# GTEC-UDC/roskfpos

Hardware: AMD Instinct MI355X
Metric: EKF predict+update steps/s at 65536 tags x 8 anchors; RMS pos err vs CPU ref (higher is better)
Workload: dtype f64 arithmetic; f64 state and covariance, f32/int32 measurements in HBM (KFPOS_STORE_MIXED)

## Files before the change

### __graft_entry__.py

```python
from __future__ import annotations

import os
import shutil
import subprocess
import sys

ROOT = os.path.dirname(os.path.abspath(__file__))
CSRC = os.path.join(ROOT, "roskfpos_amd", "csrc")
HIP_LIB = os.path.join(CSRC, "libkfpos_hip.so")
ADAPTOR_DEMO = os.path.join(CSRC, "kfpos_replay")


def _stale(target, sources):
    if not os.path.exists(target):
        return True
    mt = os.path.getmtime(target)
    return any(os.path.getmtime(s) > mt for s in sources if os.path.exists(s))


def build(force: bool = False) -> None:
    jobs = str(min(8, os.cpu_count() or 1))
    res = subprocess.run(["make", "-s", "-j", jobs, "-C", CSRC] + (["-B"] if force else []) + ["all"],
                         capture_output=True, text=True)
    if res.returncode != 0:
        sys.stderr.write(res.stdout + res.stderr)
        raise subprocess.CalledProcessError(res.returncode, res.args)
    res = subprocess.run(["make", "-s", "-C", CSRC, "check"], capture_output=True, text=True)
    if res.returncode != 0:
        sys.stderr.write(res.stdout + res.stderr)
        if os.path.exists(HIP_LIB):
            os.remove(HIP_LIB)
        raise RuntimeError("a build-time performance rule is broken (scratch inside a loop / a kernel lost its second "
                           "wavefront per SIMD / the 9-state epoch loop waits for a memory operation just issued / a trip of its gain "
                           "iteration touches memory or branches too often / its epoch loop carries a covariance across the back-edge in "
                           "registers): " + (res.stdout + res.stderr).strip())
    subprocess.check_call(["make", "-s", "-C", os.path.join(ROOT, "oracle")] + (["-B"] if force else []))
    import glob
    core_headers = sorted(glob.glob(os.path.join(CSRC, "kfpos_core*.h"))) + [os.path.join(CSRC, "kfpos_p48.h")]
    emu_dir = os.path.join(ROOT, "tests", "emu")
    emu_so = os.path.join(emu_dir, "libkfpos_emu.so")
    if force or _stale(emu_so, [os.path.join(emu_dir, "kfpos_emu.cpp")] + core_headers):
        subprocess.check_call(["g++", "-O2", "-std=c++17", "-fPIC", "-shared", "-Wno-unknown-pragmas",
                               "-o", emu_so, os.path.join(emu_dir, "kfpos_emu.cpp")])
    fake_dir = os.path.join(ROOT, "tests", "fake_rccl")
    fake_so = os.path.join(fake_dir, "libfake_rccl.so")
    if force or _stale(fake_so, [os.path.join(fake_dir, "fake_rccl.cpp")]):
        subprocess.check_call([shutil.which("hipcc") or "/opt/rocm/bin/hipcc", "-O2", "-std=c++17", "-shared", "-fPIC",
                               "-o", fake_so, os.path.join(fake_dir, "fake_rccl.cpp"), "-lrt"])
    if ROOT not in sys.path:
        sys.path.insert(0, ROOT)
    import roskfpos_amd
    from roskfpos_amd import capi
    capi.load()


def smoke() -> None:
    if ROOT not in sys.path:
        sys.path.insert(0, ROOT)
    sys.path.insert(0, os.path.join(ROOT, "oracle"))
    import numpy as np
    from roskfpos_amd import capi
    from roskfpos_amd.synth import Workload
    import oracle_py

    T, A, S = 256, 8, 12
    w = Workload(T, A)
    for model in (capi.MODEL_TOA, capi.MODEL_TOA_IMU):
        bank = capi.KfposBank(model, T, w.anchors, init_pos=w.init_positions())
        orc = oracle_py.OracleBank(model, T, w.anchors, init_pos=w.init_positions(), n_threads=4)
        err, cov = w.err_est(), w.accel_cov()
        for s in range(S):
            r, a, dt = w.ranges_mm(s), w.accel(s), w.dt_of(s)
            if model == capi.MODEL_TOA_IMU:
                bank.step_toa_imu(r, err, a, cov, dt)
                orc.step_imu(a, cov, 0.0)
                orc.step_toa(r, err, dt)
            else:
                bank.step_toa(r, err, dt)
                orc.step_toa(r, err, dt)
        x, _, _ = bank.get_state()
        xo, _ = orc.get_state()
        rms = float(np.sqrt(((x[:, :3] - xo[:, :3]) ** 2).sum(1).mean()))
        print(f"smoke model={model}: RMS position difference vs oracle = {rms:.3e} m")
        assert rms <= 1e-6, rms
        bank.close()


if __name__ == "__main__":
    build()
    if len(sys.argv) > 1 and sys.argv[1] == "smoke":
        smoke()
```

### roskfpos_amd/csrc/kfpos_core.h

```cpp
#ifndef KFPOS_CORE_H
#define KFPOS_CORE_H

#include <math.h>
#include <stdint.h>

#ifndef KFPOS_HD
#define KFPOS_HD
#endif
#define KFPOS_FN KFPOS_HD inline __attribute__((always_inline))
#if defined(__clang__)
#define KFPOS_UNROLL _Pragma("unroll")
#define KFPOS_NOUNROLL _Pragma("nounroll")
#else
#define KFPOS_UNROLL
#define KFPOS_NOUNROLL
#endif

#if defined(__HIP_DEVICE_COMPILE__)
#define KFPOS_WAVE_ALL(pred) (__all((pred) ? 1 : 0) != 0)
#else
#define KFPOS_WAVE_ALL(pred) (pred)
#endif
#if defined(__HIP_DEVICE_COMPILE__)
#define KFPOS_WAVE_ANY(pred) (__builtin_amdgcn_ballot_w64(pred) != 0)
// ... 73 lines not shown
}
KFPOS_FN void kf_sqrt_rsqrt(double x, double &d, double &invd) {
#if defined(__HIP_DEVICE_COMPILE__)
    invd = kf_rsqrt(x);
    const double s = x * invd;
    d = __builtin_fma(__builtin_fma(-s, s, x) * 0.5, invd, s);
#else
    d = sqrt(x);
    invd = 1.0 / d;
#endif
}

KFPOS_FN void kf_sqrt_rsqrt_sweep(double x, double &d, double &invd) {
#if defined(__HIP_DEVICE_COMPILE__)
    double y = __builtin_amdgcn_rsq(x);
    const double e = __builtin_fma(-(0.5 * x) * y, y, 0.5);
    y = __builtin_fma(y, e, y);
    const double s = x * y;
    d = __builtin_fma(__builtin_fma(-s, s, x) * 0.5, y, s);
    invd = y;
#else
    d = sqrt(x);
    invd = 1.0 / d;
#endif
}

KFPOS_FN double kf_mm_to_m(int32_t mm) {
#if defined(__HIP_DEVICE_COMPILE__)
    const double x = (double)mm;
    const double q = x * 0.001;
    const double r = __builtin_fma(-q, 1000.0, x);
    return __builtin_fma(r, 0.001, q);
#else
    return (double)mm / 1000;
#endif
}

KFPOS_FN bool rel_change_below(double cost, double c, double tol) {
    const double lhs = fabs(cost - c), rhs = tol * cost;
    const bool clear = cost > 0.0 && fabs(lhs - rhs) > 1e-13 * rhs;
    if (KFPOS_WAVE_ALL(clear)) return lhs < rhs;
    return lhs / cost < tol;
}

KFPOS_FN bool rel_change_below_voted(double cost, double c, double tol) {
    const double lhs = fabs(cost - c), rhs = tol * cost;
    const bool clear = cost > 0.0 && fabs(lhs - rhs) > 1e-13 * rhs;
    bool below = lhs < rhs;
    if (KFPOS_WAVE_ANY(!clear)) below = lhs / cost < tol;
    return below;
}

KFPOS_FN bool rel_change_above(double cost, double c, double tol) {
    const double lhs = fabs(cost - c), rhs = tol * cost;
    const bool clear = cost > 0.0 && fabs(lhs - rhs) > 1e-13 * rhs;
    if (KFPOS_WAVE_ALL(clear)) return lhs > rhs;
    return lhs / cost > tol;
}

KFPOS_FN double stdmax(double a, double b) { return (a < b) ? b : a; }

template <int N, bool SYMM>
struct Cov {
    static constexpr int SZ = SYMM ? N * (N + 1) / 2 : N * N;
    double a[SZ];
    KFPOS_HD static constexpr int idx(int i, int j) {
        return SYMM ? (i <= j ? i * N - i * (i - 1) / 2 + (j - i) : j * N - j * (j - 1) / 2 + (i - j))
                    : i * N + j;
    }
    KFPOS_HD double operator()(int i, int j) const { return a[idx(i, j)]; }
    KFPOS_HD double &operator()(int i, int j) { return a[idx(i, j)]; }
};

struct Params {
    const double *anchors;
    int n_anchors;
    double accel_noise, jolt, cost_threshold;
    int ignore_worst, top_n, use_init_pos;
    int ml_variant = 0;
    int use_fixed_height, imu_fixed_cov_acc, imu_fixed_cov_w;
    double px4_height, px4_arm_p1, px4_arm_p2, px4_cov_vel, px4_cov_gyro_z;
    double imu_cov_acc, imu_cov_w, mag_offset, mag_cov;
    const double *pair_anchor_tab = nullptr;
};

KFPOS_FN double sym3_cofactors(const double h[6], double c[6]) {
    c[0] = h[3] * h[5] - h[4] * h[4];
    c[1] = h[2] * h[4] - h[1] * h[5];
    c[2] = h[1] * h[4] - h[2] * h[3];
    c[3] = h[0] * h[5] - h[2] * h[2];
    c[4] = h[1] * h[2] - h[0] * h[4];
    c[5] = h[0] * h[3] - h[1] * h[1];
    return h[0] * c[0] + h[1] * c[1] + h[2] * c[2];
}
KFPOS_FN double gen3_adjugate(const double m[9], double adj[9]) {
    adj[0] = m[4] * m[8] - m[5] * m[7];
    adj[1] = m[2] * m[7] - m[1] * m[8];
    adj[2] = m[1] * m[5] - m[2] * m[4];
    adj[3] = m[5] * m[6] - m[3] * m[8];
    adj[4] = m[0] * m[8] - m[2] * m[6];
    adj[5] = m[2] * m[3] - m[0] * m[5];
    adj[6] = m[3] * m[7] - m[4] * m[6];
    adj[7] = m[1] * m[6] - m[0] * m[7];
    adj[8] = m[0] * m[4] - m[1] * m[3];
    return m[0] * adj[0] + m[1] * adj[3] + m[2] * adj[6];
}

template <int N, int K>
KFPOS_FN void gauss_solve(const double *a, const double *b, double *x) {
    double r[N][N + K];
    KFPOS_UNROLL
    for (int i = 0; i < N; ++i) {
        KFPOS_UNROLL
        for (int j = 0; j < N; ++j) r[i][j] = a[N * i + j];
        KFPOS_UNROLL
        for (int k = 0; k < K; ++k) r[i][N + k] = b[K * i + k];
    }
    KFPOS_UNROLL
    for (int c = 0; c < N; ++c) {
        KFPOS_UNROLL
        for (int i = c + 1; i < N; ++i) {
            const bool sw = fabs(r[i][c]) > fabs(r[c][c]);
            KFPOS_UNROLL
            for (int k = c; k < N + K; ++k) {
                const double tc = r[c][k], ti = r[i][k];
                r[c][k] = sw ? ti : tc;
                r[i][k] = sw ? tc : ti;
            }
        }
        const double ip = 1.0 / r[c][c];
        KFPOS_UNROLL
        for (int i = c + 1; i < N; ++i) {
            const double f = r[i][c] * ip;
            KFPOS_UNROLL
            for (int k = c + 1; k < N + K; ++k) r[i][k] -= f * r[c][k];
        }
    }
    KFPOS_UNROLL
    for (int k = 0; k < K; ++k) {
        double sol[N];
        KFPOS_UNROLL
        for (int i = N - 1; i >= 0; --i) {
            double v = r[i][N + k];
            KFPOS_UNROLL
            for (int j = i + 1; j < N; ++j) v -= r[i][j] * sol[j];
            sol[i] = v / r[i][i];
        }
        KFPOS_UNROLL
        for (int i = 0; i < N; ++i) x[K * i + k] = sol[i];
    }
}

KFPOS_FN void chol3_psd(const double m[6], double l[6], double il[3]) {
    const double REL = 1e-12;
    double d = m[0], sq, isq;
    bool ok = d > 0.0;
    kf_sqrt_rsqrt(ok ? d : 1.0, sq, isq);
    l[0] = ok ? sq : 0.0;
    il[0] = ok ? isq : 0.0;
    l[1] = m[1] * il[0];
    l[2] = m[2] * il[0];
    d = m[3] - l[1] * l[1];
    ok = d > REL * m[3];
    kf_sqrt_rsqrt(ok ? d : 1.0, sq, isq);
    l[3] = ok ? sq : 0.0;
    il[1] = ok ? isq : 0.0;
// ... 159 lines not shown
```

### roskfpos_amd/csrc/kfpos_core_imu9.h

```cpp
#ifndef KFPOS_CORE_IMU9_H
#define KFPOS_CORE_IMU9_H

namespace kfpos {

constexpr double INFO_FORM_MIN_PIVOT = 1e-7;

struct Tag9 {
    double pos[3], vel[3];
    Cov<9, true> P;
};
struct Imu {
    bool has;
    double acc[3];
    double *ci;
    int ci_stride;
    KFPOS_HD double Wi(int k) const { return ci[(6 + k) * ci_stride]; }
};

KFPOS_FN void imu_whitener(const double s[9], double *ci, int ci_stride) {
    double c00, c11, c22, i00, i11, i22;
    kf_sqrt_rsqrt(s[0], c00, i00);
    const double c10 = s[3] * i00, c20 = s[6] * i00;
    kf_sqrt_rsqrt(s[4] - c10 * c10, c11, i11);
    const double c21 = (s[7] - c20 * c10) * i11;
// ... 538 lines not shown
template <bool DIAG, bool ACC0>
KFPOS_FN void iekf9_pairs(uint64_t m, const double xhat[9], const double *binv, int binv_stride,
                          const RegScratch<8> &sc, const double *anchor_tab, const Imu &imu, int max_steps, double tol,
                          Iekf9Iter &it, Iekf9Out &o) {
    const int lane = (int)__builtin_amdgcn_mbcnt_hi(~0u, __builtin_amdgcn_mbcnt_lo(~0u, 0u));
    const int g = lane >> 1, h = lane & 1;
    const int n_surv = __popcll(m);
    bool act = g < n_surv;
    const int src = nth_set_bit(m, act ? g : 0);
    const int src4 = src << 2;
    double xh[9];
    KFPOS_UNROLL
    for (int k = 0; k < 3; ++k) {
        xh[k] = lane_pull(xhat[k], src4);
        xh[3 + k] = 0.0;
        xh[6 + k] = ACC0 ? 0.0 : lane_pull(xhat[6 + k], src4);
    }
    Iekf9Iter ct;
    KFPOS_UNROLL
    for (int k = 0; k < 6; ++k) { ct.ve[k] = lane_pull(it.ve[k], src4); ct.wl[k] = lane_pull(it.wl[k], src4); }
    ct.qd = lane_pull(it.qd, src4);
    ct.cost = lane_pull(it.cost, src4);
    Iekf9Out co;
    KFPOS_UNROLL
    for (int k = 0; k < 6; ++k) co.mrlast[k] = lane_pull(o.mrlast[k], src4);
    KFPOS_UNROLL
    for (int k = 0; k < 3; ++k) co.dlast[k] = lane_pull(o.dlast[k], src4);
    co.gain_iters = __builtin_amdgcn_ds_bpermute(src4, o.gain_iters);
    Imu ci;
    ci.has = __builtin_amdgcn_ds_bpermute(src4, imu.has ? 1 : 0) != 0;
    KFPOS_UNROLL
    for (int k = 0; k < 3; ++k) ci.acc[k] = lane_pull(imu.acc[k], src4);
    ci.ci = imu.ci + (src - lane);
    ci.ci_stride = imu.ci_stride;
    double r4[4], w4[4];
    KFPOS_UNROLL
    for (int k = 0; k < 4; ++k) {
        const double r0 = lane_pull(sc.r[k], src4), r1 = lane_pull(sc.r[4 + k], src4);
        const double w0 = lane_pull(sc.w[k], src4), w1 = lane_pull(sc.w[4 + k], src4);
        r4[k] = h ? r1 : r0;
        w4[k] = h ? w1 : w0;
    }
    const double *cbinv = binv + (src - lane);
    const double *b4 = anchor_tab + 12 * h;
    const double b0[3] = {b4[0], b4[1], b4[2]};
    while (act) {
        double bb[12];
        const int z = kf_opaque_zero();
        bb[0] = b0[0]; bb[1] = b0[1]; bb[2] = b0[2];
        KFPOS_UNROLL
        for (int k = 3; k < 12; ++k) bb[k] = b4[k + z];
        Iekf9Parked pk;
        iekf9_fetch<true, DIAG>(cbinv, binv_stride, ci, pk);
        const double p[3] = {xh[0] + ct.ve[0], xh[1] + ct.ve[1], xh[2] + ct.ve[2]};
        Sweep9 sw, other;
        iekf9_sweep4(p, r4, w4, bb, sw);
        other.c = dpp_exchange(sw.c, 0);
        KFPOS_UNROLL
        for (int k = 0; k < 6; ++k) other.m[k] = dpp_exchange(sw.m[k], 0);
        KFPOS_UNROLL
        for (int k = 0; k < 3; ++k) other.u[k] = dpp_exchange(sw.u[k], 0);
        sweep9_add(sw, other);
        iekf9_spread_reads();
        const bool more = iekf9_pass<DIAG, false>(xh, pk, ci, tol, sw, ct, co);
        act = more && co.gain_iters < max_steps;
    }
    const bool owner = (m >> lane) & 1ull;
    const int rank = __popcll(m & ((1ull << lane) - 1ull));
    const int from4 = (owner ? 2 * rank : lane) << 2;
    KFPOS_UNROLL
    for (int k = 0; k < 6; ++k) {
        const double a = lane_pull(ct.wl[k], from4), b = lane_pull(co.mrlast[k], from4);
        if (owner) { it.wl[k] = a; o.mrlast[k] = b; }
    }
    KFPOS_UNROLL
    for (int k = 0; k < 3; ++k) {
        const double a = lane_pull(co.dlast[k], from4);
        if (owner) o.dlast[k] = a;
    }
    const double cst = lane_pull(ct.cost, from4);
    const int gi = __builtin_amdgcn_ds_bpermute(from4, co.gain_iters);
    if (owner) { it.cost = cst; o.gain_iters = gi; }
}
#endif

template <bool DIAG, bool ALLIMU, bool RANGING, bool ACC0 = false, bool HOLD = true, bool SETTLE = false, class SC>
KFPOS_FN void iekf9_info(const double xhat[9], const double *binv, int binv_stride, SC &sc, const Params &pr,
                         const Imu &imu, int max_steps, double tol, Iekf9Out &o) {
    Iekf9Iter it;
    KFPOS_UNROLL
    for (int k = 0; k < 6; ++k) { it.ve[k] = 0.0; it.wl[k] = 0.0; o.mrlast[k] = 0.0; }
    it.qd = 0.0;
    it.cost = 1e20;
    o.dlast[0] = o.dlast[1] = o.dlast[2] = 0.0;
    o.gain_iters = 0;
#if defined(__HIP_DEVICE_COMPILE__)
    constexpr bool PAIRS = RANGING && SC::NA == 8 && SC::CHUNK == 0 && !SC::COOP;
    const bool pairs = PAIRS && pr.pair_anchor_tab && __builtin_amdgcn_ballot_w64(true) == ~0ull;
#endif
    bool more = true;
    int stop = max_steps;
#if defined(__HIP_DEVICE_COMPILE__)
    if (pairs) stop = 8 < max_steps ? 8 : max_steps;
#endif
    Iekf9Parked pk;
    if constexpr (HOLD) iekf9_fetch<false, DIAG, true>(binv, binv_stride, imu, pk);
#if defined(__HIP_DEVICE_COMPILE__)
    if constexpr (HOLD && SETTLE) __builtin_amdgcn_s_waitcnt(0xC07F);
#endif
    for (;;) {
        while (more && o.gain_iters < stop) {
            if constexpr (!HOLD) iekf9_fetch<false, DIAG, false>(binv, binv_stride, imu, pk);
            const double p[3] = {xhat[0] + it.ve[0], xhat[1] + it.ve[1], xhat[2] + it.ve[2]};
            Sweep9 sw;
            iekf9_sweep<RANGING>(p, sc, pr, sw);
            more = iekf9_pass<DIAG, ALLIMU>(xhat, pk, imu, tol, sw, it, o);
        }
#if defined(__HIP_DEVICE_COMPILE__)
        if constexpr (PAIRS) {
            if (pairs) {
                const uint64_t m = __builtin_amdgcn_ballot_w64(more && o.gain_iters < max_steps);
                if (m == 0) break;
                if (__popcll(m) <= 32) {
                    iekf9_pairs<DIAG, ACC0>(m, xhat, binv, binv_stride, sc, pr.pair_anchor_tab, imu, max_steps, tol, it, o);
                    break;
                }
                stop = stop + 4 < max_steps ? stop + 4 : max_steps;
                continue;
            }
        }
#endif
        break;
    }
    KFPOS_UNROLL
    for (int k = 0; k < 6; ++k) o.w[k] = it.wl[k];
    o.cost = it.cost;
}

KFPOS_FN void cov_update9(Cov<9, true> &P, const double mr[6], const double d[3], const Imu &imu) {
    Factor9 f;
    factor9(mr, d, imu, f);
    KFPOS_UNROLL
    for (int k = 0; k < 6; ++k) {
        double pt[9], s = 1.0;
        KFPOS_UNROLL
        for (int i = 0; i < 9; ++i) {
            double v = 0.0;
            KFPOS_UNROLL
            for (int l = 0; l < 6; ++l) {
                const bool nz = (l < 3 && k < 3 && l >= k) || (l >= 3 && k >= 3 && l <= k);
                if (nz) v += P(i, e9(l)) * L9(f, l, k);
            }
            pt[i] = v;
        }
        KFPOS_UNROLL
        for (int l = 0; l < 6; ++l) {
            const bool nz = (l < 3 && k < 3 && l >= k) || (l >= 3 && k >= 3 && l <= k);
            if (nz) s += L9(f, l, k) * pt[e9(l)];
        }
        const double is = kf_rcp(s);
        KFPOS_UNROLL
        for (int i = 0; i < 9; ++i) {
            const double pi = pt[i] * is;
            KFPOS_UNROLL
            for (int j = i; j < 9; ++j) P(i, j) -= pi * pt[j];
        }
    }
}

struct CovPark9 {
    double *a;
    int stride;
};

KFPOS_FN bool imu9_started(const Tag9 &tg, const Params &pr) {
    return pr.use_init_pos || !(isnan(tg.pos[0]) || isnan(tg.pos[1]));
}
template <bool RANGING, class SC>
KFPOS_FN bool imu9_ml_init(double pos[3], SC &sc, const Params &pr, int n_valid, double c[6], uint32_t &status) {
    status = 0;
    if (!RANGING) return false;
    status = ST_FEW_RANGES;
    if (n_valid < 4) return false;
    double p[3] = {1.0, 1.0, 4.0}, sse;
    set_weights_ml(sc, pr, 0ull);
    const int it = ml_estimate(p, sc, pr, 0, n_valid, sse);
    status = ST_UPDATE_SKIPPED;
    if (ml_covariance_throws(sc, pr, 0, n_valid, sse)) return false;
    if (!ml_covariance(p, sc, pr, sse, c)) return false;
    pos[0] = p[0]; pos[1] = p[1]; pos[2] = p[2];
    status = pack_status(ST_ML_INIT, 0, it, -1);
    return true;
}
KFPOS_FN void imu9_predict_state(const Tag9 &tg, double dt, double xhat[9]) {
    const double c = dt * dt / 2;
    KFPOS_UNROLL
    for (int k = 0; k < 3; ++k) {
        xhat[k] = tg.pos[k] + dt * tg.vel[k] + c * 0.0;
        xhat[3 + k] = tg.vel[k] + dt * 0.0;
        xhat[6 + k] = 0.0;
    }
}
KFPOS_FN void imu9_park(const Cov<9, true> &P, const CovPark9 &park) {
    KFPOS_UNROLL
    for (int k = 0; k < 45; ++k) park.a[k * park.stride] = P.a[k];
}
KFPOS_FN void imu9_unpark(Cov<9, true> &P, const CovPark9 &park) {
    KFPOS_UNROLL
    for (int k = 0; k < 45; ++k) P.a[k] = park.a[k * park.stride];
}
KFPOS_FN bool imu9_predict_park(Cov<9, true> &P, double dt, double jolt, const CovPark9 &park) {
    predict9(P, dt, jolt);
    Cov<6, true> B;
    KFPOS_UNROLL
    for (int i = 0; i < 6; ++i) {
        KFPOS_UNROLL
        for (int j = i; j < 6; ++j) B(i, j) = P(e9(i), e9(j));
    }
    imu9_park(P, park);
    return sym6_inverse(B, park.a + 45 * park.stride, park.stride, INFO_FORM_MIN_PIVOT);
}
template <bool RANGING, bool HOLD, bool SETTLE, class SC>
KFPOS_FN void imu9_iterate(Tag9 &tg, const double xhat[9], SC &sc, const Params &pr, const Imu &imu,
                           const CovPark9 &park, bool fast, bool invertible, Iekf9Out &o) {
    double *binv = park.a + 45 * park.stride;
    if (invertible) {
        if (fast) iekf9_info<true, true, RANGING, true, HOLD, SETTLE>(xhat, binv, park.stride, sc, pr, imu, 20, 1e-4, o);
        else iekf9_info<false, false, RANGING, true, HOLD, SETTLE>(xhat, binv, park.stride, sc, pr, imu, 20, 1e-4, o);
        imu9_unpark(tg.P, park);
    } else {
        imu9_unpark(tg.P, park);
        if (fast) iekf9<true, RANGING>(xhat, tg.P, sc, pr, imu, 20, 1e-4, o);
        else iekf9<false, RANGING>(xhat, tg.P, sc, pr, imu, 20, 1e-4, o);
    }
    KFPOS_UNROLL
    for (int i = 0; i < 6; ++i) {
        double v = 0.0;
        KFPOS_UNROLL
        for (int k = 0; k < 6; ++k) v += tg.P(i, e9(k)) * o.w[k];
        if (i < 3) tg.pos[i] = xhat[i] + v;
        else tg.vel[i - 3] = xhat[i] + v;
    }
}

template <bool RANGING, bool HOLD = true, class SC>
KFPOS_FN bool step_imu9_state(Tag9 &tg, SC &sc, const Params &pr, double dt, const Imu &imu, const CovPark9 &park,
                              bool fast, Iekf9Out &o, uint32_t &status) {
    constexpr bool has_ranging = RANGING;
    const int n_valid = has_ranging ? count_used(sc, pr, 0) : 0;
    if (!pr.use_init_pos && (isnan(tg.pos[0]) || isnan(tg.pos[1]))) {
        status = 0;
        if (!has_ranging) return false;
        status = ST_FEW_RANGES;
        if (n_valid < 4) return false;
        double p[3] = {1.0, 1.0, 4.0}, sse, c[6];
        set_weights_ml(sc, pr, 0ull);
        const int it = ml_estimate(p, sc, pr, 0, n_valid, sse);
        status = ST_UPDATE_SKIPPED;
        if (ml_covariance_throws(sc, pr, 0, n_valid, sse)) return false;
        if (!ml_covariance(p, sc, pr, sse, c)) return false;
        tg.pos[0] = p[0]; tg.pos[1] = p[1]; tg.pos[2] = p[2];
        tg.P(0, 0) = c[0]; tg.P(0, 1) = c[1]; tg.P(1, 1) = c[3];
        status = pack_status(ST_ML_INIT, 0, it, -1);
        return false;
    }
    const double c = dt * dt / 2;
    double xhat[9];
    KFPOS_UNROLL
    for (int k = 0; k < 3; ++k) {
        xhat[k] = tg.pos[k] + dt * tg.vel[k] + c * 0.0;
        xhat[3 + k] = tg.vel[k] + dt * 0.0;
        xhat[6 + k] = 0.0;
    }
    predict9(tg.P, dt, pr.jolt);
    Cov<6, true> B;
    KFPOS_UNROLL
    for (int i = 0; i < 6; ++i) {
        KFPOS_UNROLL
        for (int j = i; j < 6; ++j) B(i, j) = tg.P(e9(i), e9(j));
    }
    KFPOS_UNROLL
    for (int k = 0; k < 45; ++k) park.a[k * park.stride] = tg.P.a[k];
    double *binv = park.a + 45 * park.stride;
    const bool invertible = sym6_inverse(B, binv, park.stride, INFO_FORM_MIN_PIVOT);
    iekf9_weights(xhat, sc, pr, has_ranging, n_valid, o);
    if (o.flags & ST_UPDATE_SKIPPED) {
        KFPOS_UNROLL
        for (int k = 0; k < 45; ++k) tg.P.a[k] = park.a[k * park.stride];
        status = ST_UPDATE_SKIPPED;
        return false;
    }
    if (invertible) {
        if (fast) iekf9_info<true, true, RANGING, true, HOLD>(xhat, binv, park.stride, sc, pr, imu, 20, 1e-4, o);
        else iekf9_info<false, false, RANGING, true, HOLD>(xhat, binv, park.stride, sc, pr, imu, 20, 1e-4, o);
        KFPOS_UNROLL
        for (int k = 0; k < 45; ++k) tg.P.a[k] = park.a[k * park.stride];
    } else {
        KFPOS_UNROLL
        for (int k = 0; k < 45; ++k) tg.P.a[k] = park.a[k * park.stride];
        if (fast) iekf9<true, RANGING>(xhat, tg.P, sc, pr, imu, 20, 1e-4, o);
        else iekf9<false, RANGING>(xhat, tg.P, sc, pr, imu, 20, 1e-4, o);
    }
    KFPOS_UNROLL
    for (int i = 0; i < 6; ++i) {
        double v = 0.0;
        KFPOS_UNROLL
        for (int k = 0; k < 6; ++k) v += tg.P(i, e9(k)) * o.w[k];
        if (i < 3) tg.pos[i] = xhat[i] + v;
        else tg.vel[i - 3] = xhat[i] + v;
    }
    status = 0;
    return true;
}
KFPOS_FN bool step_imu9_head(Tag9 &tg, const Params &pr, double dt, const CovPark9 &park) {
    if (imu9_started(tg, pr)) return imu9_predict_park(tg.P, dt, pr.jolt, park);
    imu9_park(tg.P, park);
    return false;
}
template <bool RANGING, bool HOLD = true, class SC>
KFPOS_FN bool step_imu9_state_parked(Tag9 &tg, SC &sc, const Params &pr, double dt, const Imu &imu,
                                     const CovPark9 &park, bool fast, bool invertible, Iekf9Out &o, uint32_t &status) {
    constexpr bool has_ranging = RANGING;
    const int n_valid = has_ranging ? count_used(sc, pr, 0) : 0;
    if (!imu9_started(tg, pr)) {
        double c[6];
        if (imu9_ml_init<RANGING>(tg.pos, sc, pr, n_valid, c, status)) {
            park.a[Cov<9, true>::idx(0, 0) * park.stride] = c[0];
            park.a[Cov<9, true>::idx(0, 1) * park.stride] = c[1];
            park.a[Cov<9, true>::idx(1, 1) * park.stride] = c[3];
        }
        imu9_unpark(tg.P, park);
        return false;
    }
    double xhat[9];
    imu9_predict_state(tg, dt, xhat);
    iekf9_weights(xhat, sc, pr, has_ranging, n_valid, o);
    if (o.flags & ST_UPDATE_SKIPPED) {
        imu9_unpark(tg.P, park);
        status = ST_UPDATE_SKIPPED;
        return false;
    }
    imu9_iterate<RANGING, HOLD, true>(tg, xhat, sc, pr, imu, park, fast, invertible, o);
    status = 0;
    return true;
}
KFPOS_FN uint32_t step_imu9_cov(Tag9 &tg, const Iekf9Out &o, const Imu &imu) {
    cov_update9(tg.P, o.mrlast, o.dlast, imu);
    return pack_status(o.flags, o.gain_iters, o.ml_iters, -1);
}
template <bool RANGING, class SC>
KFPOS_FN uint32_t step_imu9(Tag9 &tg, SC &sc, const Params &pr, double dt, const Imu &imu, const CovPark9 &park) {
    Iekf9Out o;
    uint32_t status;
    if (!step_imu9_state<RANGING>(tg, sc, pr, dt, imu, park, false, o, status)) return status;
    return step_imu9_cov(tg, o, imu);
}

KFPOS_FN void pose9(const Tag9 &tg, double t, double jolt, double pos[3], double vel[3], double cov[9]) {
    const double c = t * t / 2, t3 = (t * t * t) / 6;
    KFPOS_UNROLL
    for (int i = 0; i < 3; ++i) {
        pos[i] = tg.pos[i] + t * tg.vel[i];
        vel[i] = tg.vel[i];
        KFPOS_UNROLL
        for (int j = 0; j < 3; ++j) {
            const Cov<9, true> &P = tg.P;
            const double xpp = P(i, j) + t * P(3 + i, j) + c * P(6 + i, j);
            const double xpv = P(i, 3 + j) + t * P(3 + i, 3 + j) + c * P(6 + i, 3 + j);
            const double xpa = P(i, 6 + j) + t * P(3 + i, 6 + j) + c * P(6 + i, 6 + j);
            cov[3 * i + j] = xpp + t * xpv + c * xpa + (i == j ? jolt * t3 * t3 : 0.0);
        }
    }
}

}
#endif
```

### roskfpos_amd/csrc/kfpos_hip.hip

```cpp
#include <algorithm>
#include <cmath>
#include <cstdio>
#include <cstdlib>
#include <cstring>
#include <new>
#include <string>
#include <type_traits>
#include <vector>

#include "kfpos_kernels.h"

std::string &kfpos_error_text() {
    thread_local std::string text;
    return text;
}

namespace {

#define g_err (kfpos_error_text())

#define HIPCHK(expr)                                                                              \
    do {                                                                                          \
        hipError_t e_ = (expr);                                                                   \
        if (e_ != hipSuccess) {                                                                   \
// ... 224 lines not shown
using DevScope = KfposDevScope;

inline int pidx(const kfpos_handle *h, int i, int j) {
    if (h->full) return i * h->n + j;
    const int N = h->n;
    if (i > j) { const int tt = i; i = j; j = tt; }
    return i * N - i * (i - 1) / 2 + (j - i);
}

}

extern "C" {

const char *kfpos_last_error(void) { return g_err.c_str(); }
const char *kfpos_strerror(int code) {
    switch (code) {
    case KFPOS_OK: return "ok";
    case KFPOS_ERR_ARG: return "invalid argument";
    case KFPOS_ERR_HIP: return "HIP runtime error";
    case KFPOS_ERR_NO_DEVICE: return "no usable GPU";
    case KFPOS_ERR_MODEL: return "call not defined for this model";
    case KFPOS_ERR_STATE: return "call out of sequence";
    case KFPOS_ERR_COMM: return "RCCL error";
    default: return "unknown error";
    }
}
int kfpos_version(void) { return KFPOS_VERSION; }

int kfpos_create(const kfpos_config *cfg, kfpos_handle **out) {
    if (!cfg || !out) return KFPOS_ERR_ARG;
    *out = nullptr;
    g_err.clear();
    auto bad = [](const char *why) {
        g_err = why;
        return KFPOS_ERR_ARG;
    };
    if (cfg->model != KFPOS_MODEL_TOA && cfg->model != KFPOS_MODEL_TOA_IMU && cfg->model != KFPOS_MODEL_ML &&
        cfg->model != KFPOS_MODEL_PLANAR)
        return bad("kfpos_config.model is not one of KFPOS_MODEL_*");
    if (cfg->storage != KFPOS_STORE_F64 && cfg->storage != KFPOS_STORE_F32 && cfg->storage != KFPOS_STORE_MIXED &&
        cfg->storage != KFPOS_STORE_P48)
        return bad("kfpos_config.storage is not one of KFPOS_STORE_*");
    if (cfg->n_tags < 1) return bad("kfpos_config.n_tags must be >= 1");
    if (cfg->max_anchors < 1 || cfg->max_anchors > KFPOS_MAX_ANCHORS)
        return bad("kfpos_config.max_anchors must be 1..64 (MAX_NUM_ANCS, Posgenerator.h:74)");
    if (cfg->top_n < 0) return bad("kfpos_config.top_n must be >= 0");
    if (cfg->ml_variant != KFPOS_ML_NORMAL && cfg->ml_variant != KFPOS_ML_IGNORE_N && cfg->ml_variant != KFPOS_ML_BEST)
        return bad("kfpos_config.ml_variant is not one of KFPOS_ML_*");
    if (cfg->ml_variant != KFPOS_ML_NORMAL && cfg->model != KFPOS_MODEL_ML)
        return bad("kfpos_config.ml_variant belongs to KFPOS_MODEL_ML (MLLocation's variants, MLLocation.h:5-7)");
    if ((cfg->model == KFPOS_MODEL_TOA_IMU && (cfg->top_n || cfg->ignore_worst)) ||
        (cfg->model == KFPOS_MODEL_ML && cfg->ignore_worst) ||
        (cfg->model == KFPOS_MODEL_PLANAR && (cfg->top_n || cfg->ignore_worst)))
        return bad("ignore_worst exists for the 6-state filter only, top_n for the 6-state filter and the ML estimator");
    int ndev = 0;
    if (hipGetDeviceCount(&ndev) != hipSuccess || ndev <= 0 || cfg->device < 0 || cfg->device >= ndev) {
        g_err = "no HIP device";
        return KFPOS_ERR_NO_DEVICE;
    }
    DevScope dev_(cfg->device);
    kfpos_handle *h = new (std::nothrow) kfpos_handle();
    if (!h) return KFPOS_ERR_ARG;
    h->cfg = *cfg;
    h->n = cfg->model == KFPOS_MODEL_TOA_IMU ? 9 : (cfg->model == KFPOS_MODEL_ML ? 3 : (cfg->model == KFPOS_MODEL_PLANAR ? 8 : 6));
    h->full = (cfg->model == KFPOS_MODEL_TOA && !cfg->use_init_pos) ? 1 : 0;
    h->psz = h->full ? h->n * h->n : h->n * (h->n + 1) / 2;
    h->rsz = cfg->storage == KFPOS_STORE_F32 ? 4 : (cfg->storage == KFPOS_STORE_P48 ? 6 : 8);
    h->msz = cfg->storage == KFPOS_STORE_F64 ? 8 : 4;
    h->A = 0;
    h->have_anchors = false;
    h->stepped = false;
    {
        const char *g = getenv("KFPOS_GENERIC_KERNEL");
        h->force_generic = g && g[0] == '1';
        if (h->full && cfg->ignore_worst && cfg->storage == KFPOS_STORE_P48) h->force_generic = true;
        {
            hipDeviceProp_t prop;
            const char *ow = getenv("KFPOS_ONE_WAVE_BUILD");
            h->two_waves = false;
            if (!(ow && ow[0] == '1') && hipGetDeviceProperties(&prop, cfg->device) == hipSuccess)
                h->two_waves = ((size_t)cfg->n_tags + WAVE - 1) / WAVE > (size_t)prop.multiProcessorCount * 4;
        }
        const char *np = getenv("KFPOS_PAIR9");
        h->pair9 = np && np[0] == '1';
        const char *nd = getenv("KFPOS_IMU9_DIAG");
        h->imu9_diag = !(nd && nd[0] == '0');
        const char *nc = getenv("KFPOS_NO_COOP");
        h->coop = !(nc && nc[0] == '1') && !h->force_generic && cfg->model == KFPOS_MODEL_TOA && cfg->use_init_pos &&
                  !cfg->ignore_worst && !cfg->top_n && cfg->max_anchors <= COOP_LANES && cfg->n_tags <= 8192;
        const char *c = getenv("KFPOS_TRACE_CHUNK_STEPS");
        int n = c ? atoi(c) : KFPOS_TRACE_CHUNK;
        h->trace_chunk = n < 1 ? 1 : (n > KFPOS_TRACE_CHUNK ? KFPOS_TRACE_CHUNK : n);
    }
    std::memset(h->anchors, 0, sizeof(h->anchors));
    const size_t T = cfg->n_tags, A = cfg->max_anchors, r = h->rsz, m = h->msz;
#define ALLOC(ptr, bytes)                                                     \
    do {                                                                      \
        hipError_t e_ = hipMalloc((void **)&(ptr), (bytes));                  \
        if (e_ != hipSuccess) {                                               \
            g_err = std::string("hipMalloc: ") + hipGetErrorString(e_);       \
            kfpos_destroy(h);                                                 \
            return KFPOS_ERR_HIP;                                             \
        }                                                                     \
        (void)hipMemset((ptr), 0, (bytes));                                   \
    } while (0)
    ALLOC(h->d_pos, 3 * T * sizeof(double));
    ALLOC(h->d_P, h->psz * T * r);
    ALLOC(h->d_flags, T * sizeof(uint32_t));
    if (h->n == 3) ALLOC(h->d_vel, 3 * T * sizeof(double));
    if (h->n == 8) {
        ALLOC(h->d_vel, 4 * T * sizeof(double));
        ALLOC(h->d_latch, LATCH_ROWS * T * sizeof(double));
        ALLOC(h->d_sensor, 24 * T * sizeof(double));
    }
    if (h->n == 9) {
        ALLOC(h->d_vel, 3 * T * sizeof(double));
        ALLOC(h->d_imu_acc, 3 * T * m);
        ALLOC(h->d_imu_cov, 6 * T * m);
        ALLOC(h->d_accel, 3 * T * m);
        ALLOC(h->d_cov, 9 * T * m);
    }
    ALLOC(h->d_ranges, A * T * sizeof(int32_t));
    ALLOC(h->d_err, A * T * m);
    ALLOC(h->d_dt, T * sizeof(double));
    ALLOC(h->d_out, 15 * T * sizeof(double));
    ALLOC(h->d_status, T * sizeof(uint32_t));
#undef ALLOC
    if (hipEventCreate(&h->ev0) != hipSuccess || hipEventCreate(&h->ev1) != hipSuccess) {
        g_err = "hipEventCreate failed";
        kfpos_destroy(h);
        return KFPOS_ERR_HIP;
    }
    if (T * A <= small_bank_limit()) {
        size_t off = 0;
        auto region = [&](size_t bytes) { const size_t o = off; off += (bytes + 255) & ~(size_t)255; return o; };
        h->sm_ranges = region(A * T * sizeof(int32_t));
        h->sm_err = region(A * T * m);
        h->sm_accel = region(3 * T * m);
        h->sm_cov = region(9 * T * m);
        h->sm_dt = region(T * sizeof(double));
        h->sm_sensor = region(24 * T * sizeof(double));
        h->sm_status = region(T * sizeof(uint32_t));
        h->sm_out = region((size_t)(15 + h->n + h->n * h->n) * T * sizeof(double));
        void *hp = nullptr, *dp = nullptr;
        if (hipHostMalloc(&hp, off, hipHostMallocMapped) != hipSuccess || hipHostGetDevicePointer(&dp, hp, 0) != hipSuccess) {
            g_err = "hipHostMalloc(mapped block of a small bank) failed";
            if (hp) (void)hipHostFree(hp);
            kfpos_destroy(h);
            return KFPOS_ERR_HIP;
        }
        std::memset(hp, 0, off);
        h->sm_h = (unsigned char *)hp;
        h->sm_bytes = off;
        h->sm_d = (unsigned char *)dp;
    }
    const bool parks = cfg->model == KFPOS_MODEL_PLANAR || (cfg->model == KFPOS_MODEL_TOA && h->full);
    if (cfg->model == KFPOS_MODEL_TOA_IMU && lds_bytes(h) + park9_bytes() > 64 * 1024) {
        hipError_t e_ = hipFuncSetAttribute((const void *)step_kernel(h), hipFuncAttributeMaxDynamicSharedMemorySize,
                                            (int)(lds_bytes(h) + park9_bytes()));
        if (e_ != hipSuccess) {
            g_err = std::string("hipFuncSetAttribute: ") + hipGetErrorString(e_);
            kfpos_destroy(h);
            return KFPOS_ERR_HIP;
        }
    } else if (lds_bytes(h) + (parks ? park_bytes() : 0) > 64 * 1024) {
        hipError_t e_ = hipFuncSetAttribute((const void *)step_kernel(h), hipFuncAttributeMaxDynamicSharedMemorySize,
                                            (int)(lds_bytes(h) + (h->full ? park_bytes() : 0)));
// ... 1986 lines not shown
```

### roskfpos_amd/csrc/kfpos_k_imu9.hip

```cpp
#include "kfpos_kernels.h"

namespace {

template <typename W>
__device__ inline void in_agpr(W &w) {
    static_assert(sizeof(W) == 4, "one register");
    asm volatile("" : "+a"(w));
}

__device__ inline void forget(double &v) { asm volatile("" : "=v"(v)); }

template <typename REAL, typename MREAL, int AS, bool RANGING = true>
__global__ __launch_bounds__(WAVE) void k_step_imu9(const KArgs a) {
    extern __shared__ double lds[];
    const int lane = threadIdx.x;
    const size_t t = (size_t)blockIdx.x * WAVE + lane;
    if (t >= (size_t)a.T) return;
    const size_t T = a.T;
    const uint32_t t32 = (uint32_t)t;
    Params pr = make_params(a);
    constexpr bool has_ranging = RANGING;
    constexpr bool AHEAD = sizeof(MREAL) == 4 && !std::is_same<REAL, float>::value;
    const bool fresh_imu = a.mode != MODE_TOA;
    constexpr int NA = AS > 0 ? AS : 1;
    double dt_tag = a.dt_shared;
    if (a.n_steps == 1 && a.dt) {
        dt_tag = a.dt[t32];
        if (dt_tag < 0.0) {
            skipped_lane(a, t, true);
            return;
        }
    }

    uint32_t fl = a.flags[t32];
    RawEpoch<MREAL, NA> raw;
    RawImu<MREAL> rawi;
    if constexpr (AS > 0) {
        if (has_ranging) fetch_epoch<MREAL, AS>(a, t, 0, raw);
    }
    Tag9 tg;
#pragma unroll
    for (int k = 0; k < 3; ++k) {
        tg.pos[k] = (a.pos + k * T)[t32];
        tg.vel[k] = (a.vel + k * T)[t32];
    }
    const CovPark9 park{lds + ((AS == 0 && has_ranging) ? 3 * (size_t)a.A * WAVE : 0) + lane, WAVE};
    Imu imu;
    imu.has = false;
    imu.ci = park.a + 66 * WAVE;
    imu.ci_stride = WAVE;
    if constexpr (AS == 8 && RANGING) {
        if (a.pair9) {
            double *tab = lds + 78 * WAVE;
#pragma unroll
            for (int k = 0; k < 24; ++k) tab[k] = a.anchors[k];
            pr.pair_anchor_tab = tab;
        }
    }
    double cv[9] = {1, 0, 0, 0, 1, 0, 0, 0, 1};
    MREAL rawc[9];
    if (fresh_imu) {
        fetch_imu<MREAL>(a, t, 0, rawi);
        fetch_imu_cov<MREAL>(a, t, 0, rawc);
    } else if (fl & FL_HAS_IMU) {
        imu.has = true;
#pragma unroll
        for (int k = 0; k < 3; ++k) imu.acc[k] = ldrow<MREAL>(a.imu_acc, k, T, t32);
        cv[0] = ldrow<MREAL>(a.imu_cov, 0, T, t32);
        cv[3] = ldrow<MREAL>(a.imu_cov, 1, T, t32);
        cv[4] = ldrow<MREAL>(a.imu_cov, 2, T, t32);
        cv[6] = ldrow<MREAL>(a.imu_cov, 3, T, t32);
        cv[7] = ldrow<MREAL>(a.imu_cov, 4, T, t32);
        cv[8] = ldrow<MREAL>(a.imu_cov, 5, T, t32);
    }
#pragma unroll
    for (int k = 0; k < 45; ++k) tg.P.a[k] = ldcov<REAL>(a.P, k, 45, T, t32);
    if (fresh_imu) {
        imu.has = true;
#pragma unroll
        for (int k = 0; k < 9; ++k) cv[k] = (double)rawc[k];
        if (a.latch) latch_imu_cov<MREAL>(a, T, t32, cv);
    }
    if (imu.has) imu_whitener(cv, imu.ci, imu.ci_stride);
    bool diag = false;
    if (a.imu9_diag) {
        const bool mine = !imu.has || (imu.Wi(1) == 0.0 && imu.Wi(2) == 0.0 && imu.Wi(4) == 0.0);
        diag = __builtin_amdgcn_ballot_w64(mine) == __builtin_amdgcn_ballot_w64(true);
    }
    const bool fast = imu9_fast(diag, imu.has);

    const bool multi = a.n_steps > 1;
    double dt_next = multi ? a.dt_steps[0] : dt_tag;
    constexpr bool IMU_WITH_EPOCH = AHEAD && AS > 0 && RANGING;
    constexpr bool ROTATE = IMU_WITH_EPOCH && AS == 8 && std::is_same<REAL, double>::value;

    __builtin_amdgcn_s_waitcnt(0x0F70);
    uint32_t s = 0;
    if constexpr (ROTATE) {
        bool invertible = step_imu9_head(tg, pr, dt_next, park);
        double latched[3] = {0.0, 0.0, 0.0};
        if (!fresh_imu && imu.has) {
#pragma unroll
            for (int k = 0; k < 3; ++k) latched[k] = imu.acc[k];
        }
        for (int e = 0; e < a.n_steps; ++e) {
            const double dt = dt_next;
            const bool more = e + 1 < a.n_steps;
            if (multi && more) dt_next = a.dt_steps[opaque_uniform(e + 1)];
#pragma unroll
            for (int k = 0; k < NA; ++k) { in_agpr(raw.mm[k]); in_agpr(raw.e[k]); }
            if (fresh_imu) {
#pragma unroll
                for (int k = 0; k < 3; ++k) in_agpr(rawi.acc[k]);
            }
#pragma unroll
            for (int k = 0; k < 3; ++k) imu.acc[k] = fresh_imu ? (double)rawi.acc[k] : latched[k];
            RegScratch<NA> sc;
            unpack_epoch<MREAL, NA>(raw, sc);
#pragma unroll
            for (int k = 0; k < NA; ++k) { kfpos::kf_pin(sc.r[k]); kfpos::kf_pin(sc.e[k]); }
#pragma unroll
            for (int k = 0; k < 3; ++k) kfpos::kf_pin(imu.acc[k]);
            asm volatile("" ::: "memory");
            const int ahead = opaque_uniform(more ? e + 1 : e);
            fetch_epoch<MREAL, NA>(a, opaque_lane(t), ahead, raw);
            if (fresh_imu) fetch_imu<MREAL>(a, opaque_lane(t), ahead, rawi);
            Iekf9Out o;
#pragma unroll
            for (int k = 0; k < 6; ++k) { forget(o.w[k]); forget(o.mrlast[k]); }
#pragma unroll
            for (int k = 0; k < 3; ++k) forget(o.dlast[k]);
            const bool update = step_imu9_state_parked<RANGING>(tg, sc, pr, dt, imu, park, fast, invertible, o, s);
            if (a.traj) {
#pragma unroll
                for (int k = 0; k < 3; ++k) (a.traj + ((size_t)opaque_uniform(e) * 3 + k) * T)[t32] = tg.pos[k];
            }
            if (update) s = step_imu9_cov(tg, o, imu);
            if (more) {
                static_assert(!cov_is_rounded<REAL>(), "a rounded covariance is rounded here, in front of the head");
                invertible = step_imu9_head(tg, pr, dt_next, park);
#pragma unroll
                for (int k = 0; k < 45; ++k) forget(tg.P.a[k]);
            }
        }
    } else
    for (int e = 0; e < a.n_steps; ++e) {
        const double dt = dt_next;
        if (multi && e + 1 < a.n_steps) dt_next = a.dt_steps[opaque_uniform(e + 1)];
        if (fresh_imu) {
#pragma unroll
            for (int k = 0; k < 3; ++k) imu.acc[k] = (double)rawi.acc[k];
            if constexpr (AHEAD && !IMU_WITH_EPOCH) {
                if (e + 1 < a.n_steps) fetch_imu<MREAL>(a, opaque_lane(t), opaque_uniform(e + 1), rawi);
            }
        }
        Iekf9Out o;
        auto finish = [&](bool update) {
            if (a.traj) {
#pragma unroll
                for (int k = 0; k < 3; ++k) (a.traj + ((size_t)opaque_uniform(e) * 3 + k) * T)[t32] = tg.pos[k];
            }
            if (update) s = step_imu9_cov(tg, o, imu);
        };
        if constexpr (AS > 0) {
            RegScratch<AS> sc;
            if (has_ranging) {
                unpack_epoch<MREAL, AS>(raw, sc);
                if (e + 1 < a.n_steps) {
                    if constexpr (AHEAD) {
                        fetch_epoch<MREAL, AS>(a, opaque_lane(t), opaque_uniform(e + 1), raw);
                        if constexpr (IMU_WITH_EPOCH) {
                            if (fresh_imu) fetch_imu<MREAL>(a, opaque_lane(t), opaque_uniform(e + 1), rawi);
                        }
                    }
                }
            } else {
#pragma unroll
                for (int k = 0; k < AS; ++k) sc.r[k] = sc.e[k] = sc.w[k] = 0.0;
            }
            finish(step_imu9_state<RANGING>(tg, sc, pr, dt, imu, park, fast, o, s));
            if constexpr (!AHEAD) {
                if (e + 1 < a.n_steps) {
                    if (fresh_imu) fetch_imu<MREAL>(a, opaque_lane(t), opaque_uniform(e + 1), rawi);
                    if (has_ranging) fetch_epoch<MREAL, AS>(a, opaque_lane(t), opaque_uniform(e + 1), raw);
                }
            }
        } else {
            Scratch sc{nullptr, nullptr, nullptr, WAVE};
            if (has_ranging) sc = stage_epoch_lds<MREAL>(a, lds, lane, t, opaque_uniform(e));
            finish(step_imu9_state<RANGING>(tg, sc, pr, dt, imu, park, fast, o, s));
            if constexpr (!AHEAD) {
                if (e + 1 < a.n_steps && fresh_imu) fetch_imu<MREAL>(a, opaque_lane(t), opaque_uniform(e + 1), rawi);
            }
        }
        if constexpr (cov_is_rounded<REAL>()) {
            if (e + 1 < a.n_steps) {
#pragma unroll
                for (int k = 0; k < 45; ++k) tg.P.a[k] = round_cov<REAL>(tg.P.a[k]);
            }
        }
    }

    if (fresh_imu && a.latch) {
#pragma unroll
        for (int k = 0; k < 3; ++k) strow<MREAL>(a.imu_acc, k, T, t32, imu.acc[k]);
        fl |= FL_HAS_IMU;
    }
    bool fin = true;
#pragma unroll
    for (int k = 0; k < 3; ++k) {
        (a.pos + k * T)[t32] = tg.pos[k];
        (a.vel + k * T)[t32] = tg.vel[k];
        fin &= isfinite(tg.pos[k]) & isfinite(tg.vel[k]);
    }
#pragma unroll
    for (int k = 0; k < 45; ++k) {
        stcov<REAL>(a.P, k, 45, T, t32, tg.P.a[k]);
        fin &= isfinite(tg.P.a[k]);
    }
    const bool waiting = !a.use_init_pos && isnan(tg.pos[0]);
    if (!fin && !waiting) s |= ST_NONFINITE;
    a.flags[t32] = fl | FL_STARTED;
    if (a.status) a.status[t32] = s;
}

}

template <typename REAL, typename MREAL>
static kfpos_k::step_kernel_t imu9_of(int as, bool ranging) {
    if (!ranging) return k_step_imu9<REAL, MREAL, 0, false>;
    if (as == 8) return k_step_imu9<REAL, MREAL, 8>;
    return k_step_imu9<REAL, MREAL, 0>;
}
kfpos_k::step_kernel_t kfpos_k::imu9_kernel(int st, int as, bool ranging) {
    return KFPOS_BY_STORAGE(st, imu9_of, as, ranging);
}
```

Measured before the change: 2.164 billion.

## Add register-held paired-lane IEKF tail for mixed-storage 8-anchor IMU kernel

Adds a variant of the paired-lane gain iteration in which two lanes share one straggling tag, each sweeping four anchors. Anchor coordinates, ranges, weights and the parked inverse are held in registers instead of being read from an LDS anchor table. Partial sums are combined with DPP exchanges, and results are written back only for lanes whose iteration count changed. The pair mode is now on by default for mixed and P48 storage. This is meant to cut divergence cost in the iteration tail when few lanes remain active, at the price of extra register pressure and cross-lane shuffles.

```diff
diff --git a/__graft_entry__.py b/__graft_entry__.py
--- a/__graft_entry__.py
+++ b/__graft_entry__.py
@@ -32,7 +32,7 @@
             os.remove(HIP_LIB)
         raise RuntimeError("a build-time performance rule is broken (scratch inside a loop / a kernel lost its second "
                            "wavefront per SIMD / the 9-state epoch loop waits for a memory operation just issued / a trip of its gain "
-                           "iteration touches memory or branches too often / its epoch loop carries a covariance across the back-edge in "
+                           "iteration, per lane or in pairs, touches memory or branches too often / its epoch loop carries a covariance across the back-edge in "
                            "registers): " + (res.stdout + res.stderr).strip())
     subprocess.check_call(["make", "-s", "-C", os.path.join(ROOT, "oracle")] + (["-B"] if force else []))
     import glob
diff --git a/roskfpos_amd/csrc/kfpos_core.h b/roskfpos_amd/csrc/kfpos_core.h
--- a/roskfpos_amd/csrc/kfpos_core.h
+++ b/roskfpos_amd/csrc/kfpos_core.h
@@ -179,6 +179,7 @@
     double px4_height, px4_arm_p1, px4_arm_p2, px4_cov_vel, px4_cov_gyro_z;
     double imu_cov_acc, imu_cov_w, mag_offset, mag_cov;
     const double *pair_anchor_tab = nullptr;
+    bool pair9 = false;
 };
 
 KFPOS_FN double sym3_cofactors(const double h[6], double c[6]) {
diff --git a/roskfpos_amd/csrc/kfpos_core_imu9.h b/roskfpos_amd/csrc/kfpos_core_imu9.h
--- a/roskfpos_amd/csrc/kfpos_core_imu9.h
+++ b/roskfpos_amd/csrc/kfpos_core_imu9.h
@@ -644,9 +644,98 @@
     const int gi = __builtin_amdgcn_ds_bpermute(from4, co.gain_iters);
     if (owner) { it.cost = cst; o.gain_iters = gi; }
 }
+template <bool DIAG, bool ALLIMU, bool ACC0>
+KFPOS_FN void iekf9_pairs_held(uint64_t m, const double xhat[9], const double *binv, int binv_stride,
+                               const RegScratch<8> &sc, const Params &pr, const Imu &imu, int max_steps, double tol,
+                               Iekf9Iter &it, Iekf9Out &o) {
+    const int lane = (int)__builtin_amdgcn_mbcnt_hi(~0u, __builtin_amdgcn_mbcnt_lo(~0u, 0u));
+    const int g = lane >> 1;
+    const bool h = lane & 1;
+    const int n_surv = __popcll(m);
+    bool act = g < n_surv;
+    const int src = nth_set_bit(m, act ? g : 0);
+    const int src4 = src << 2;
+    Imu ci;
+    ci.ci = imu.ci + (src - lane);
+    ci.ci_stride = imu.ci_stride;
+    Iekf9Parked pk;
+    iekf9_fetch<false, DIAG, false>(binv + (src - lane), binv_stride, ci, pk);
+    double xh[9];
+    KFPOS_UNROLL
+    for (int k = 0; k < 3; ++k) {
+        xh[k] = lane_pull(xhat[k], src4);
+        xh[3 + k] = 0.0;
+        xh[6 + k] = ACC0 ? 0.0 : lane_pull(xhat[6 + k], src4);
+    }
+    Iekf9Iter ct;
+    KFPOS_UNROLL
+    for (int k = 0; k < 6; ++k) { ct.ve[k] = lane_pull(it.ve[k], src4); ct.wl[k] = 0.0; }
+    ct.qd = lane_pull(it.qd, src4);
+    ct.cost = lane_pull(it.cost, src4);
+    Iekf9Out co;
+    KFPOS_UNROLL
+    for (int k = 0; k < 6; ++k) co.mrlast[k] = 0.0;
+    KFPOS_UNROLL
+    for (int k = 0; k < 3; ++k) co.dlast[k] = 0.0;
+    co.gain_iters = __builtin_amdgcn_ds_bpermute(src4, o.gain_iters);
+    ci.has = ALLIMU || __builtin_amdgcn_ds_bpermute(src4, imu.has ? 1 : 0) != 0;
+    KFPOS_UNROLL
+    for (int k = 0; k < 3; ++k) ci.acc[k] = lane_pull(imu.acc[k], src4);
+    double r4[4], w4[4], bb[12];
+    KFPOS_UNROLL
+    for (int k = 0; k < 4; ++k) {
+        const double r0 = lane_pull(sc.r[k], src4), r1 = lane_pull(sc.r[4 + k], src4);
+        const double w0 = lane_pull(sc.w[k], src4), w1 = lane_pull(sc.w[4 + k], src4);
+        r4[k] = h ? r1 : r0;
+        w4[k] = h ? w1 : w0;
+    }
+    KFPOS_UNROLL
+    for (int k = 0; k < 12; ++k) {
+        bb[k] = h ? pr.anchors[12 + k] : pr.anchors[k];
+        kf_pin(bb[k]);
+    }
+    KFPOS_UNROLL
+    for (int k = 0; k < 21; ++k) kf_pin(pk.binv[k]);
+    KFPOS_UNROLL
+    for (int k = 0; k < 6; ++k) {
+        if (!DIAG || k == 0 || k == 3 || k == 5) kf_pin(pk.wi[k]);
+    }
+    __builtin_amdgcn_s_waitcnt(0xC07F);
+    while (act) {
+        const double p[3] = {xh[0] + ct.ve[0], xh[1] + ct.ve[1], xh[2] + ct.ve[2]};
+        Sweep9 sw, other;
+        iekf9_sweep4(p, r4, w4, bb, sw);
+        other.c = dpp_exchange(sw.c, 0);
+        KFPOS_UNROLL
+        for (int k = 0; k < 6; ++k) other.m[k] = dpp_exchange(sw.m[k], 0);
+        KFPOS_UNROLL
+        for (int k = 0; k < 3; ++k) other.u[k] = dpp_exchange(sw.u[k], 0);
+        sweep9_add(sw, other);
+        const bool more = iekf9_pass<DIAG, ALLIMU>(xh, pk, ci, tol, sw, ct, co);
+        act = more && co.gain_iters < max_steps;
+    }
+    const bool owner = (m >> lane) & 1ull;
+    const int rank = __popcll(m & ((1ull << lane) - 1ull));
+    const int from4 = (owner ? 2 * rank : lane) << 2;
+    const int gi = __builtin_amdgcn_ds_bpermute(from4, co.gain_iters);
+    const bool moved = owner && gi != o.gain_iters;
+    KFPOS_UNROLL
+    for (int k = 0; k < 6; ++k) {
+        const double a = lane_pull(ct.wl[k], from4), b = lane_pull(co.mrlast[k], from4);
+        if (moved) { it.wl[k] = a; o.mrlast[k] = b; }
+    }
+    KFPOS_UNROLL
+    for (int k = 0; k < 3; ++k) {
+        const double a = lane_pull(co.dlast[k], from4);
+        if (moved) o.dlast[k] = a;
+    }
+    const double cst = lane_pull(ct.cost, from4);
+    if (moved) { it.cost = cst; o.gain_iters = gi; }
+}
 #endif
 
-template <bool DIAG, bool ALLIMU, bool RANGING, bool ACC0 = false, bool HOLD = true, bool SETTLE = false, class SC>
+template <bool DIAG, bool ALLIMU, bool RANGING, bool ACC0 = false, bool HOLD = true, bool SETTLE = false,
+          bool TAIL = false, class SC>
 KFPOS_FN void iekf9_info(const double xhat[9], const double *binv, int binv_stride, SC &sc, const Params &pr,
                          const Imu &imu, int max_steps, double tol, Iekf9Out &o) {
     Iekf9Iter it;
@@ -658,7 +747,7 @@
     o.gain_iters = 0;
 #if defined(__HIP_DEVICE_COMPILE__)
     constexpr bool PAIRS = RANGING && SC::NA == 8 && SC::CHUNK == 0 && !SC::COOP;
-    const bool pairs = PAIRS && pr.pair_anchor_tab && __builtin_amdgcn_ballot_w64(true) == ~0ull;
+    const bool pairs = PAIRS && (TAIL ? pr.pair9 : pr.pair_anchor_tab != nullptr) && __builtin_amdgcn_ballot_w64(true) == ~0ull;
 #endif
     bool more = true;
     int stop = max_steps;
@@ -684,7 +773,8 @@
                 const uint64_t m = __builtin_amdgcn_ballot_w64(more && o.gain_iters < max_steps);
                 if (m == 0) break;
                 if (__popcll(m) <= 32) {
-                    iekf9_pairs<DIAG, ACC0>(m, xhat, binv, binv_stride, sc, pr.pair_anchor_tab, imu, max_steps, tol, it, o);
+                    if constexpr (TAIL) iekf9_pairs_held<DIAG, ALLIMU, ACC0>(m, xhat, binv, binv_stride, sc, pr, imu, max_steps, tol, it, o);
+                    else iekf9_pairs<DIAG, ACC0>(m, xhat, binv, binv_stride, sc, pr.pair_anchor_tab, imu, max_steps, tol, it, o);
                     break;
                 }
                 stop = stop + 4 < max_steps ? stop + 4 : max_steps;
@@ -782,13 +872,13 @@
     imu9_park(P, park);
     return sym6_inverse(B, park.a + 45 * park.stride, park.stride, INFO_FORM_MIN_PIVOT);
 }
-template <bool RANGING, bool HOLD, bool SETTLE, class SC>
+template <bool RANGING, bool HOLD, bool SETTLE, bool TAIL, class SC>
 KFPOS_FN void imu9_iterate(Tag9 &tg, const double xhat[9], SC &sc, const Params &pr, const Imu &imu,
                            const CovPark9 &park, bool fast, bool invertible, Iekf9Out &o) {
     double *binv = park.a + 45 * park.stride;
     if (invertible) {
-        if (fast) iekf9_info<true, true, RANGING, true, HOLD, SETTLE>(xhat, binv, park.stride, sc, pr, imu, 20, 1e-4, o);
-        else iekf9_info<false, false, RANGING, true, HOLD, SETTLE>(xhat, binv, park.stride, sc, pr, imu, 20, 1e-4, o);
+        if (fast) iekf9_info<true, true, RANGING, true, HOLD, SETTLE, TAIL>(xhat, binv, park.stride, sc, pr, imu, 20, 1e-4, o);
+        else iekf9_info<false, false, RANGING, true, HOLD, SETTLE, TAIL>(xhat, binv, park.stride, sc, pr, imu, 20, 1e-4, o);
         imu9_unpark(tg.P, park);
     } else {
         imu9_unpark(tg.P, park);
@@ -805,7 +895,7 @@
     }
 }
 
-template <bool RANGING, bool HOLD = true, class SC>
+template <bool RANGING, bool HOLD = true, bool TAIL = false, class SC>
 KFPOS_FN bool step_imu9_state(Tag9 &tg, SC &sc, const Params &pr, double dt, const Imu &imu, const CovPark9 &park,
                               bool fast, Iekf9Out &o, uint32_t &status) {
     constexpr bool has_ranging = RANGING;
@@ -853,8 +943,8 @@
         return false;
     }
     if (invertible) {
-        if (fast) iekf9_info<true, true, RANGING, true, HOLD>(xhat, binv, park.stride, sc, pr, imu, 20, 1e-4, o);
-        else iekf9_info<false, false, RANGING, true, HOLD>(xhat, binv, park.stride, sc, pr, imu, 20, 1e-4, o);
+        if (fast) iekf9_info<true, true, RANGING, true, HOLD, false, TAIL>(xhat, binv, park.stride, sc, pr, imu, 20, 1e-4, o);
+        else iekf9_info<false, false, RANGING, true, HOLD, false, TAIL>(xhat, binv, park.stride, sc, pr, imu, 20, 1e-4, o);
         KFPOS_UNROLL
         for (int k = 0; k < 45; ++k) tg.P.a[k] = park.a[k * park.stride];
     } else {
@@ -879,7 +969,7 @@
     imu9_park(tg.P, park);
     return false;
 }
-template <bool RANGING, bool HOLD = true, class SC>
+template <bool RANGING, bool HOLD = true, bool TAIL = false, class SC>
 KFPOS_FN bool step_imu9_state_parked(Tag9 &tg, SC &sc, const Params &pr, double dt, const Imu &imu,
                                      const CovPark9 &park, bool fast, bool invertible, Iekf9Out &o, uint32_t &status) {
     constexpr bool has_ranging = RANGING;
@@ -902,7 +992,7 @@
         status = ST_UPDATE_SKIPPED;
         return false;
     }
-    imu9_iterate<RANGING, HOLD, true>(tg, xhat, sc, pr, imu, park, fast, invertible, o);
+    imu9_iterate<RANGING, HOLD, true, TAIL>(tg, xhat, sc, pr, imu, park, fast, invertible, o);
     status = 0;
     return true;
 }
diff --git a/roskfpos_amd/csrc/kfpos_hip.hip b/roskfpos_amd/csrc/kfpos_hip.hip
--- a/roskfpos_amd/csrc/kfpos_hip.hip
+++ b/roskfpos_amd/csrc/kfpos_hip.hip
@@ -330,7 +330,8 @@
                 h->two_waves = ((size_t)cfg->n_tags + WAVE - 1) / WAVE > (size_t)prop.multiProcessorCount * 4;
         }
         const char *np = getenv("KFPOS_PAIR9");
-        h->pair9 = np && np[0] == '1';
+        h->pair9 = np && np[0] ? np[0] == '1'
+                               : (cfg->storage == KFPOS_STORE_MIXED || cfg->storage == KFPOS_STORE_P48);
         const char *nd = getenv("KFPOS_IMU9_DIAG");
         h->imu9_diag = !(nd && nd[0] == '0');
         const char *nc = getenv("KFPOS_NO_COOP");
diff --git a/roskfpos_amd/csrc/kfpos_k_imu9.hip b/roskfpos_amd/csrc/kfpos_k_imu9.hip
--- a/roskfpos_amd/csrc/kfpos_k_imu9.hip
+++ b/roskfpos_amd/csrc/kfpos_k_imu9.hip
@@ -49,7 +49,9 @@
     imu.has = false;
     imu.ci = park.a + 66 * WAVE;
     imu.ci_stride = WAVE;
-    if constexpr (AS == 8 && RANGING) {
+    constexpr bool TAIL = AS == 8 && RANGING && sizeof(MREAL) == 4 && !std::is_same<REAL, float>::value;
+    if constexpr (TAIL) pr.pair9 = a.pair9 != 0;
+    else if constexpr (AS == 8 && RANGING) {
         if (a.pair9) {
             double *tab = lds + 78 * WAVE;
 #pragma unroll
@@ -130,7 +132,7 @@
             for (int k = 0; k < 6; ++k) { forget(o.w[k]); forget(o.mrlast[k]); }
 #pragma unroll
             for (int k = 0; k < 3; ++k) forget(o.dlast[k]);
-            const bool update = step_imu9_state_parked<RANGING>(tg, sc, pr, dt, imu, park, fast, invertible, o, s);
+            const bool update = step_imu9_state_parked<RANGING, true, TAIL>(tg, sc, pr, dt, imu, park, fast, invertible, o, s);
             if (a.traj) {
 #pragma unroll
                 for (int k = 0; k < 3; ++k) (a.traj + ((size_t)opaque_uniform(e) * 3 + k) * T)[t32] = tg.pos[k];
@@ -178,7 +180,7 @@
 #pragma unroll
                 for (int k = 0; k < AS; ++k) sc.r[k] = sc.e[k] = sc.w[k] = 0.0;
             }
-            finish(step_imu9_state<RANGING>(tg, sc, pr, dt, imu, park, fast, o, s));
+            finish(step_imu9_state<RANGING, true, TAIL>(tg, sc, pr, dt, imu, park, fast, o, s));
             if constexpr (!AHEAD) {
                 if (e + 1 < a.n_steps) {
                     if (fresh_imu) fetch_imu<MREAL>(a, opaque_lane(t), opaque_uniform(e + 1), rawi);
@@ -188,7 +190,7 @@
         } else {
             Scratch sc{nullptr, nullptr, nullptr, WAVE};
             if (has_ranging) sc = stage_epoch_lds<MREAL>(a, lds, lane, t, opaque_uniform(e));
-            finish(step_imu9_state<RANGING>(tg, sc, pr, dt, imu, park, fast, o, s));
+            finish(step_imu9_state<RANGING, true, TAIL>(tg, sc, pr, dt, imu, park, fast, o, s));
             if constexpr (!AHEAD) {
                 if (e + 1 < a.n_steps && fresh_imu) fetch_imu<MREAL>(a, opaque_lane(t), opaque_uniform(e + 1), rawi);
             }
```

Result: faster. 2.194 billion (median of 6 runs) (+1.4%).
